# umutdundar99/progressive-stable-diffusion

Measured on AMD Instinct MI355X. Metric: images/sec at 512x512, 50 DDIM steps, bs/GPU=4, higher is better.
Workload: dtype f16; 1 GPU; 512x512, 50 DDIM steps, bs=4/GPU, delta-steer lambda=3.0, routing gates on, conditioning prep + VAE decode included; global_batch=4, parallelism=batch-shard x1 + 1 all-gather of uint8 frames

## Files before the change

progressive-stable-diffusion_amd/csrc/attn2_fused.hip:

```cpp
#include "dadd_common.h"
#include "igemm_args.h"

namespace {

constexpr int BK = 64, NS = 384, BN2 = 160;
constexpr int B1_BYTES = NS * BK * 2;
constexpr int P_STRIDE = 896;
constexpr int B2_BYTES = BN2 * BK * 2;
template <int BM> constexpr int a_bytes() { return BM * BK * 2; }
template <int BM> constexpr int stage1() { return a_bytes<BM>() + B1_BYTES; }
template <int BM> constexpr int p_bytes() { return BM * P_STRIDE; }
template <int BM> constexpr int nst2() { return p_bytes<BM>() + 4 * B2_BYTES <= 160 * 1024 - 1024 ? 4 : 2; }
template <int BM> constexpr int smem_bytes() {
  return (p_bytes<BM>() + nst2<BM>() * B2_BYTES) > 2 * stage1<BM>() ? (p_bytes<BM>() + nst2<BM>() * B2_BYTES) : 2 * stage1<BM>();
}

typedef __attribute__((address_space(3))) void* lptr_t;
constexpr unsigned OOB = 0x80000000u;

struct Attn2Args {
  const half_t* x;
  const half_t* mcat;
  const half_t* vw;
  const float* bias;
  const half_t* residual;
  half_t* out;
  float* ln_stats;
  const float* ln_in;
  const float* ln_c1;
  const float* ln_d;
  float ln_eps;
  int ln_parts;
  int B, HW, C;
};

__device__ __forceinline__ int lds_off(int row, int chunk) {
  return (row * 8 + (chunk ^ ((row >> 1) & 7))) * 8;
}

template <int BM>
__global__ __launch_bounds__(256, 1) void attn2_fused_kernel(const Attn2Args p) {
#if defined(__HIP_DEVICE_COMPILE__)
  constexpr int MI = BM / 32;
  constexpr int WMR = BM / 2;
  constexpr int NXP = BM / 32;
  constexpr int A_BYTES = a_bytes<BM>(), STAGE1 = stage1<BM>(), P_BYTES = p_bytes<BM>();
  extern __shared__ __attribute__((aligned(1024))) char smem[];
  const int t = threadIdx.x, lane = t & 63;
  const int wave = __builtin_amdgcn_readfirstlane(t >> 6);
  const int wm = wave >> 1, wn = wave & 1;
  const int tile = xcd_remap(blockIdx.x, gridDim.x);
  const int m0 = tile * BM;
  const int b = m0 / p.HW;
  const int C = p.C;
  const int nk1 = C / BK;
  const int lrow = lane >> 3, lch = lane & 7;
  const int fq = lane >> 4, mc = lane & 15, g = fq;

  const __amdgpu_buffer_rsrc_t rsX =
      __builtin_amdgcn_make_buffer_rsrc((void*)p.x, 0, (int)((size_t)p.B * p.HW * C * 2), 0x00020000);
  const __amdgpu_buffer_rsrc_t rsM = __builtin_amdgcn_make_buffer_rsrc(
      (void*)(p.mcat + (size_t)b * NS * C), 0, NS * C * 2, 0x00020000);
  unsigned xv[NXP], mv[12];
#pragma unroll
  for (int i = 0; i < NXP; ++i) {
    const int row = (i * 4 + wave) * 8 + lrow;
    xv[i] = (unsigned)(((size_t)(m0 + row) * C + (lch ^ ((row >> 1) & 7)) * 8) * 2);
  }
#pragma unroll
  for (int j = 0; j < 12; ++j) {
    const int row = (j * 4 + wave) * 8 + lrow;
    mv[j] = (unsigned)(((size_t)row * C + (lch ^ ((row >> 1) & 7)) * 8) * 2);
  }
  auto issue1 = [&](int kt, int stage) {
    char* sa = smem + stage * STAGE1 + wave * 1024;
    const unsigned ko = (unsigned)(kt * BK * 2);
#pragma unroll
    for (int i = 0; i < NXP; ++i)
      __builtin_amdgcn_raw_ptr_buffer_load_lds(rsX, (lptr_t)(sa + i * 4096), 16, xv[i], ko, 0, 0);
#pragma unroll
    for (int j = 0; j < 12; ++j)
      __builtin_amdgcn_raw_ptr_buffer_load_lds(rsM, (lptr_t)(sa + A_BYTES + j * 4096), 16, mv[j], ko, 0, 0);
  };

  f4 acc[12][MI];
#pragma unroll
  for (int j = 0; j < 12; ++j)
#pragma unroll
    for (int i = 0; i < MI; ++i) acc[j][i] = f4{0.f, 0.f, 0.f, 0.f};
  const bool fold = p.ln_in != nullptr;
  float lmu[MI], lrs[MI];
#pragma unroll
  for (int i = 0; i < MI; ++i) lmu[i] = 0.f, lrs[i] = 1.f;
  if (fold) {
    const dadd_f2* st = reinterpret_cast<const dadd_f2*>(p.ln_in);
    const size_t mtot = (size_t)p.B * p.HW;
    float sa[MI], sq[MI];
#pragma unroll
    for (int i = 0; i < MI; ++i) sa[i] = sq[i] = 0.f;
    for (int pp = 0; pp < p.ln_parts; ++pp)
#pragma unroll
      for (int i = 0; i < MI; ++i) {
        const dadd_f2 v = st[(size_t)pp * mtot + m0 + wm * WMR + i * 16 + mc];
        sa[i] += v[0];
        sq[i] += v[1];
      }
    const float inv = __builtin_amdgcn_rcpf((float)C);
#pragma unroll
    for (int i = 0; i < MI; ++i) {
      const float mu = sa[i] * inv;
      lmu[i] = mu;
      lrs[i] = rsqrtf(fmaxf(sq[i] * inv - mu * mu, 0.f) + p.ln_eps);
    }
  }
  int fa[2], fb[2];
#pragma unroll
  for (int s = 0; s < 2; ++s) {
    fa[s] = lds_off(wm * WMR + mc, s * 4 + fq) * 2;
    fb[s] = A_BYTES + lds_off(wn * 192 + mc, s * 4 + fq) * 2;
  }
  issue1(0, 0);
  for (int kt = 0; kt < nk1; ++kt) {
    asm volatile("s_waitcnt vmcnt(0)" ::: "memory");
    __syncthreads();
    if (kt + 1 < nk1) issue1(kt + 1, (kt + 1) & 1);
    const char* st = smem + (kt & 1) * STAGE1;
#pragma unroll
    for (int s = 0; s < 2; ++s) {
      h8 xa[MI], wb[12];
#pragma unroll
      for (int i = 0; i < MI; ++i) xa[i] = *reinterpret_cast<const h8*>(st + fa[s] + i * 2048);
#pragma unroll
      for (int j = 0; j < 12; ++j) wb[j] = *reinterpret_cast<const h8*>(st + fb[s] + j * 2048);
#pragma unroll
      for (int j = 0; j < 12; ++j)
#pragma unroll
        for (int i = 0; i < MI; ++i)
          acc[j][i] = __builtin_amdgcn_mfma_f32_16x16x32_f16(wb[j], xa[i], acc[j][i], 0, 0, 0);
    }
  }
  f4 fc1[12], fd[12];
  if (fold) {
#pragma unroll
    for (int j = 0; j < 12; ++j) {
      const int k = wn * 192 + j * 16 + g * 4;
      fc1[j] = *reinterpret_cast<const f4*>(p.ln_c1 + (size_t)b * NS + k);
      fd[j] = *reinterpret_cast<const f4*>(p.ln_d + (size_t)b * NS + k);
    }
  }
  __syncthreads();

  const int nt2 = C / BN2;
  const int nk2 = NS / BK;
  const int n_it2 = nt2 * nk2;
  const __amdgpu_buffer_rsrc_t rsV = __builtin_amdgcn_make_buffer_rsrc(
      (void*)(p.vw + (size_t)b * C * NS), 0, C * NS * 2, 0x00020000);
  unsigned vv[5];
#pragma unroll
  for (int j = 0; j < 5; ++j) {
    const int row = (j * 4 + wave) * 8 + lrow;
    vv[j] = (unsigned)(((size_t)row * NS + (lch ^ ((row >> 1) & 7)) * 8) * 2);
  }
  auto issue2 = [&](int it, int stage) {
    const int nt = it / nk2, kt = it - nt * nk2;
    char* sa = smem + P_BYTES + stage * B2_BYTES + wave * 1024;
    const unsigned so = (unsigned)(((size_t)nt * BN2 * NS + kt * BK) * 2);
#pragma unroll
    for (int j = 0; j < 5; ++j)
      __builtin_amdgcn_raw_ptr_buffer_load_lds(rsV, (lptr_t)(sa + j * 4096), 16, vv[j], so, 0, 0);
  };
  constexpr int NST2 = nst2<BM>();
  issue2(0, 0);
  if constexpr (NST2 == 4) {
    if (1 < n_it2) issue2(1, 1);
    if (2 < n_it2) issue2(2, 2);
  }

#pragma unroll
  for (int i = 0; i < MI; ++i) {
    const int row = wm * WMR + i * 16 + mc;
    char* prow = smem + row * P_STRIDE;
    const int swz = (row >> 1) & 7;
#pragma unroll
    for (int j = 0; j < 12; ++j) {
      f4 v = acc[j][i];
      if (fold) v = lrs[i] * (v - lmu[i] * fc1[j]) + fd[j];
      float mx = fmaxf(fmaxf(v[0], v[1]), fmaxf(v[2], v[3]));
      mx = dadd_max_x16x32(mx);
      const float e0 = __builtin_amdgcn_exp2f(v[0] - mx), e1 = __builtin_amdgcn_exp2f(v[1] - mx);
      const float e2 = __builtin_amdgcn_exp2f(v[2] - mx), e3 = __builtin_amdgcn_exp2f(v[3] - mx);
      float sum = (e0 + e1) + (e2 + e3);
      sum = dadd_sum_x16x32(sum);
      const float inv = __builtin_amdgcn_rcpf(sum);
      const h4 o = {(half_t)(e0 * inv), (half_t)(e1 * inv), (half_t)(e2 * inv), (half_t)(e3 * inv)};
      const int k = wn * 192 + j * 16 + g * 4;
      const int seg = k >> 6, ch = (k & 63) >> 3;
      *reinterpret_cast<h4*>(prow + seg * 128 + ((ch ^ swz) << 4) + (k & 7) * 2) = o;
    }
  }

  const int fp0 = (wm * WMR + mc) * P_STRIDE;
  const int pswz = ((wm * WMR + mc) >> 1) & 7;
  const int swb = wn * 80 + mc;
  const int fv0 = (swb * 8 + (fq ^ ((swb >> 1) & 7))) * 16;
  f4 acc2[5][MI];
  for (int it = 0; it < n_it2; ++it) {
    const int nt = it / nk2, kt = it - nt * nk2;
    if (kt == 0) {
#pragma unroll
      for (int j = 0; j < 5; ++j)
#pragma unroll
        for (int i = 0; i < MI; ++i) acc2[j][i] = f4{0.f, 0.f, 0.f, 0.f};
    }
    if constexpr (NST2 == 4) {
      const int younger = min(2, n_it2 - 1 - it);
      if (younger == 2) asm volatile("s_waitcnt vmcnt(10)" ::: "memory");
      else if (younger == 1) asm volatile("s_waitcnt vmcnt(5)" ::: "memory");
      else asm volatile("s_waitcnt vmcnt(0)" ::: "memory");
    } else {
      asm volatile("s_waitcnt vmcnt(0)" ::: "memory");
    }
    __syncthreads();
    if (it + NST2 - 1 < n_it2) issue2(it + NST2 - 1, (it + NST2 - 1) & (NST2 - 1));
    const char* vt = smem + P_BYTES + (it & (NST2 - 1)) * B2_BYTES;
#pragma unroll
    for (int s = 0; s < 2; ++s) {
      h8 pa[MI], wb[5];
#pragma unroll
      for (int i = 0; i < MI; ++i)
        pa[i] = *reinterpret_cast<const h8*>(smem + fp0 + i * 16 * P_STRIDE + kt * 128 + (((s * 4 + fq) ^ pswz) << 4));
#pragma unroll
      for (int j = 0; j < 5; ++j) wb[j] = *reinterpret_cast<const h8*>(vt + (fv0 ^ (s * 64)) + j * 2048);
#pragma unroll
      for (int j = 0; j < 5; ++j)
#pragma unroll
        for (int i = 0; i < MI; ++i)
          acc2[j][i] = __builtin_amdgcn_mfma_f32_16x16x32_f16(wb[j], pa[i], acc2[j][i], 0, 0, 0);
    }
    if (kt == nk2 - 1) {
      f4 bias4[5];
      h4 res4[5][MI];
#pragma unroll
      for (int j = 0; j < 5; ++j) {
        const int n = nt * BN2 + wn * 80 + j * 16 + g * 4;
        bias4[j] = p.bias ? *reinterpret_cast<const f4*>(p.bias + n) : f4{0.f, 0.f, 0.f, 0.f};
#pragma unroll
        for (int i = 0; i < MI; ++i)
          res4[j][i] = *reinterpret_cast<const h4*>(p.residual + ((size_t)m0 + wm * WMR + i * 16 + mc) * C + n);
      }
#pragma unroll
      for (int i = 0; i < MI; ++i) {
        const size_t m = (size_t)m0 + wm * WMR + i * 16 + mc;
        float rs1 = 0.f, rs2 = 0.f;
#pragma unroll
        for (int j = 0; j < 5; ++j) {
          const int n = nt * BN2 + wn * 80 + j * 16 + g * 4;
          const f4 v = acc2[j][i] + bias4[j];
          const h4 rv = res4[j][i];
          const h4 o = {(half_t)(v[0] + (float)rv[0]), (half_t)(v[1] + (float)rv[1]),
                        (half_t)(v[2] + (float)rv[2]), (half_t)(v[3] + (float)rv[3])};
          *reinterpret_cast<h4*>(p.out + m * C + n) = o;
#pragma unroll
          for (int r = 0; r < 4; ++r) {
            const float f = (float)o[r];
            rs1 += f;
            rs2 = fmaf(f, f, rs2);
          }
        }
        if (p.ln_stats) {
          rs1 = dadd_sum_x16x32(rs1);
          rs2 = dadd_sum_x16x32(rs2);
          if (g == 0)
            reinterpret_cast<dadd_f2*>(p.ln_stats)[(size_t)(nt * 2 + wn) * ((size_t)p.B * p.HW) + m] = dadd_f2{rs1, rs2};
        }
      }
    }
  }
#endif
}

}

int g_attn2_cus = 0;

int dadd_init_attn2_fused() {
  DADD_HIP(hipFuncSetAttribute(reinterpret_cast<const void*>(&attn2_fused_kernel<128>),
                               hipFuncAttributeMaxDynamicSharedMemorySize, smem_bytes<128>()));
  DADD_HIP(hipFuncSetAttribute(reinterpret_cast<const void*>(&attn2_fused_kernel<64>),
                               hipFuncAttributeMaxDynamicSharedMemorySize, smem_bytes<64>()));
  int dev = 0;
  DADD_HIP(hipGetDevice(&dev));
  DADD_HIP(hipDeviceGetAttribute(&g_attn2_cus, hipDeviceAttributeMultiprocessorCount, dev));
  return DADD_OK;
}

extern "C" int dadd_attn2_fused_f16(const void* x, const void* mcat, const void* vw, const float* bias,
                                    const void* residual, void* out, float* ln_stats_out, const float* ln_stats_in,
                                    int ln_parts_in, const float* ln_c1, const float* ln_d, float ln_eps, int B, int HW,
                                    int C, void* stream) {
  DADD_REQUIRE(x && mcat && vw && residual && out, "attn2_fused: null pointer");
  DADD_REQUIRE(B > 0 && HW > 0 && HW % 128 == 0, "attn2_fused: H*W=%d must be a multiple of 128", HW);
  DADD_REQUIRE(C > 0 && C % BN2 == 0 && C % BK == 0, "attn2_fused: C=%d must be a multiple of 320", C);
  DADD_REQUIRE((size_t)B * HW * C * 2 < 0x7FF00000ull, "attn2_fused: activation larger than the 2 GiB buffer window");
  DADD_REQUIRE(dadd_aligned16(x) && dadd_aligned16(mcat) && dadd_aligned16(vw) && dadd_aligned16(residual) &&
                   dadd_aligned16(out) && (!bias || dadd_aligned16(bias)),
// ... 29 lines not shown
```

progressive-stable-diffusion_amd/csrc/elementwise.hip:

```cpp
#include "dadd_common.h"

namespace {

#ifndef DADD_BF16
__global__ __launch_bounds__(256) void pack_kernel(const float* __restrict__ x, half_t* __restrict__ out,
                                                   int B, int C, int HW, float scale,
                                                   const float* __restrict__ mat,
                                                   const float* __restrict__ vec) {
  const size_t total = (size_t)B * HW;
  for (size_t i = (size_t)blockIdx.x * 256 + threadIdx.x; i < total; i += (size_t)gridDim.x * 256) {
    const size_t b = i / HW, pix = i - b * HW;
    float v[8], o[8];
#pragma unroll
    for (int c = 0; c < 8; ++c) v[c] = (c < C) ? x[(b * C + c) * HW + pix] * scale : 0.f;
    if (mat) {
#pragma unroll
      for (int c = 0; c < 8; ++c) {
        float a = 0.f;
        if (c < C) {
          a = vec ? vec[c] : 0.f;
          for (int k = 0; k < C; ++k) a += mat[c * C + k] * v[k];
        }
        o[c] = a;
      }
    } else {
#pragma unroll
      for (int c = 0; c < 8; ++c) o[c] = v[c];
    }
    h8 r;
#pragma unroll
    for (int c = 0; c < 8; ++c) r[c] = (half_t)o[c];
    *reinterpret_cast<h8*>(out + i * 8) = r;
  }
}

__global__ __launch_bounds__(256) void conv_cin8_kernel(const half_t* __restrict__ x,
                                                        const half_t* __restrict__ w,
                                                        const float* __restrict__ bias,
                                                        half_t* __restrict__ out, int B, int H, int W,
                                                        int Cout) {
  const int npix = B * H * W;
  const int pix = blockIdx.x * 256 + threadIdx.x;
  const int co0 = blockIdx.y * 8;
  if (pix >= npix) return;
  const int b = pix / (H * W), rem = pix - b * H * W, oy = rem / W, ox = rem - oy * W;
  float acc[8];
#pragma unroll
  for (int o = 0; o < 8; ++o) acc[o] = bias ? bias[co0 + o] : 0.f;
#pragma unroll
  for (int tap = 0; tap < 9; ++tap) {
    const int iy = oy + tap / 3 - 1, ix = ox + tap % 3 - 1;
    if (iy < 0 || iy >= H || ix < 0 || ix >= W) continue;
    const h8 xv = *reinterpret_cast<const h8*>(x + ((size_t)(b * H + iy) * W + ix) * 8);
#pragma unroll
    for (int o = 0; o < 8; ++o) {
      const h8 wv = *reinterpret_cast<const h8*>(w + ((size_t)(co0 + o) * 9 + tap) * 8);
#pragma unroll
      for (int c = 0; c < 8; ++c) acc[o] += (float)xv[c] * (float)wv[c];
    }
  }
  h8 r;
#pragma unroll
  for (int o = 0; o < 8; ++o) r[o] = (half_t)acc[o];
  *reinterpret_cast<h8*>(out + (size_t)pix * Cout + co0) = r;
}

#endif

__global__ __launch_bounds__(256) void conv_in_nchw_kernel(const float* __restrict__ x, const half_t* __restrict__ w,
                                                           const float* __restrict__ bias, half_t* __restrict__ out,
                                                           int B, int C, int H, int W, int Cout) {
  typedef half_t ci_h2 __attribute__((ext_vector_type(2)));
  const int HW = H * W, npix = B * HW;
  const int pix = blockIdx.x * 256 + threadIdx.x;
  const int co0 = blockIdx.y * 8;
  if (pix >= npix) return;
  const int b = pix / HW, rem = pix - b * HW, oy = rem / W, ox = rem - oy * W;
  ci_h2 x01[9], x23[9];
#pragma unroll
  for (int tap = 0; tap < 9; ++tap) {
    const int iy = oy + tap / 3 - 1, ix = ox + tap % 3 - 1;
    const bool ok = iy >= 0 && iy < H && ix >= 0 && ix < W;
    const float* xp = x + (size_t)b * C * HW + (ok ? iy * W + ix : rem);
    float v[4];
#pragma unroll
    for (int c = 0; c < 4; ++c) v[c] = (c < C && ok) ? xp[(size_t)c * HW] : 0.f;
    x01[tap] = ci_h2{(half_t)v[0], (half_t)v[1]};
    x23[tap] = ci_h2{(half_t)v[2], (half_t)v[3]};
  }
  h8 r;
#pragma unroll
  for (int o = 0; o < 8; ++o) {
    float acc = bias ? bias[co0 + o] : 0.f;
#pragma unroll
    for (int tap = 0; tap < 9; ++tap) {
      const h4 wv = *reinterpret_cast<const h4*>(w + ((size_t)(co0 + o) * 9 + tap) * 8);
      acc = dadd_fdot2(x01[tap], ci_h2{wv[0], wv[1]}, acc);
      acc = dadd_fdot2(x23[tap], ci_h2{wv[2], wv[3]}, acc);
    }
    r[o] = (half_t)acc;
  }
  *reinterpret_cast<h8*>(out + (size_t)pix * Cout + co0) = r;
}

template <int CG>
__global__ __launch_bounds__(256) void conv_in_nchw_gn_kernel(const float* __restrict__ x, const half_t* __restrict__ w,
                                                              const float* __restrict__ bias, half_t* __restrict__ out,
                                                              float* __restrict__ gn_ws, int B, int C, int H, int W, int Cout) {
  typedef half_t ci_h2 __attribute__((ext_vector_type(2)));
  static_assert((4 * CG) % 8 == 0, "four groups must be whole 8-channel stores");
  __shared__ float red[4][8];
  const int HW = H * W;
  const int pix = blockIdx.x * 256 + threadIdx.x;
  const int co0 = blockIdx.y * 4 * CG;
  const int b = pix / HW, rem = pix - b * HW, oy = rem / W, ox = rem - oy * W;
  ci_h2 x01[9], x23[9];
#pragma unroll
  for (int tap = 0; tap < 9; ++tap) {
    const int iy = oy + tap / 3 - 1, ix = ox + tap % 3 - 1;
    const bool ok = iy >= 0 && iy < H && ix >= 0 && ix < W;
    const float* xp = x + (size_t)b * C * HW + (ok ? iy * W + ix : rem);
    float v[4];
#pragma unroll
    for (int c = 0; c < 4; ++c) v[c] = (c < C && ok) ? xp[(size_t)c * HW] : 0.f;
    x01[tap] = ci_h2{(half_t)v[0], (half_t)v[1]};
    x23[tap] = ci_h2{(half_t)v[2], (half_t)v[3]};
  }
  float st[8] = {0.f, 0.f, 0.f, 0.f, 0.f, 0.f, 0.f, 0.f};
#pragma unroll
  for (int o8 = 0; o8 < 4 * CG / 8; ++o8) {
    h8 r;
#pragma unroll
    for (int o = 0; o < 8; ++o) {
      const int co = co0 + o8 * 8 + o;
      float acc = bias ? bias[co] : 0.f;
#pragma unroll
      for (int tap = 0; tap < 9; ++tap) {
        const h4 wv = *reinterpret_cast<const h4*>(w + ((size_t)co * 9 + tap) * 8);
        acc = dadd_fdot2(x01[tap], ci_h2{wv[0], wv[1]}, acc);
        acc = dadd_fdot2(x23[tap], ci_h2{wv[2], wv[3]}, acc);
      }
      r[o] = (half_t)acc;
      const float f = (float)r[o];
      const int g = (o8 * 8 + o) / CG;
      st[2 * g] += f;
      st[2 * g + 1] += f * f;
    }
    *reinterpret_cast<h8*>(out + (size_t)pix * Cout + co0 + o8 * 8) = r;
  }
#pragma unroll
  for (int i = 0; i < 8; ++i) st[i] = wave_sum(st[i]);
  const int lane = threadIdx.x & 63, wave = threadIdx.x >> 6;
  if (lane == 0) {
#pragma unroll
    for (int i = 0; i < 8; ++i) red[wave][i] = st[i];
  }
  __syncthreads();
  if (threadIdx.x < 8) {
    const int i = threadIdx.x;
    const float v = (red[0][i] + red[1][i]) + (red[2][i] + red[3][i]);
    const int chunk = (blockIdx.x * 256 - b * HW) >> 8, nchunk = HW >> 8;
    gn_ws[(((size_t)b * nchunk + chunk) * 32 + blockIdx.y * 4 + (i >> 1)) * 2 + (i & 1)] = v;
  }
}

typedef half_t cc_h2 __attribute__((ext_vector_type(2)));
__global__ __launch_bounds__(256) void conv_cout4_kernel(const half_t* __restrict__ x,
                                                         const half_t* __restrict__ w,
                                                         const float* __restrict__ bias,
                                                         float* __restrict__ out, int B, int H, int W,
                                                         int C, int Cout, int mode,
                                                         const float* __restrict__ coef) {
#pragma clang fp contract(off)
  extern __shared__ __attribute__((aligned(16))) char cc_smem[];
  half_t* ws = reinterpret_cast<half_t*>(cc_smem);
  const int wtot = Cout * 9 * C;
  for (int i = threadIdx.x * 8; i < wtot; i += 256 * 8) *reinterpret_cast<h8*>(ws + i) = *reinterpret_cast<const h8*>(w + i);
  __syncthreads();
  const int npix = B * H * W, HW = H * W;
  const int sub = threadIdx.x & 15;
  const int nchunk = C >> 3;
  int pixs[2], bb[2], oy[2], ox[2];
  bool live[2];
#pragma unroll
  for (int q = 0; q < 2; ++q) {
    int pix = blockIdx.x * 32 + q * 16 + (threadIdx.x >> 4);
    live[q] = pix < npix;
    if (!live[q]) pix = npix - 1;
    pixs[q] = pix;
    bb[q] = pix / HW;
    const int rem = pix - bb[q] * HW;
    oy[q] = rem / W;
    ox[q] = rem - oy[q] * W;
  }
  float a0[4] = {0.f, 0.f, 0.f, 0.f}, a1[4] = {0.f, 0.f, 0.f, 0.f};
  const h8 zero8 = {0, 0, 0, 0, 0, 0, 0, 0};
  for (int ch = sub; ch < nchunk; ch += 16) {
    h8 xv[2][9];
#pragma unroll
    for (int q = 0; q < 2; ++q)
#pragma unroll
      for (int tap = 0; tap < 9; ++tap) {
        const int iy = oy[q] + tap / 3 - 1, ix = ox[q] + tap % 3 - 1;
        const bool ok = iy >= 0 && iy < H && ix >= 0 && ix < W;
        const half_t* xp = x + ((size_t)(bb[q] * H + (ok ? iy : oy[q])) * W + (ok ? ix : ox[q])) * C + ch * 8;
        const h8 v = *reinterpret_cast<const h8*>(xp);
        xv[q][tap] = ok ? v : zero8;
      }
#pragma unroll
    for (int tap = 0; tap < 9; ++tap)
#pragma unroll
      for (int o = 0; o < 4; ++o) {
        if (o < Cout) {
          const h8 wv = *reinterpret_cast<const h8*>(ws + (o * 9 + tap) * C + ch * 8);
#pragma unroll
          for (int c = 0; c < 4; ++c) {
            const cc_h2 wp = {wv[2 * c], wv[2 * c + 1]};
            a0[o] = dadd_fdot2(cc_h2{xv[0][tap][2 * c], xv[0][tap][2 * c + 1]}, wp, a0[o]);
            a1[o] = dadd_fdot2(cc_h2{xv[1][tap][2 * c], xv[1][tap][2 * c + 1]}, wp, a1[o]);
          }
        }
      }
  }
#pragma unroll
  for (int o = 0; o < 4; ++o) {
#pragma unroll
    for (int s = 8; s > 0; s >>= 1) {
      a0[o] += __shfl_xor(a0[o], s, 64);
      a1[o] += __shfl_xor(a1[o], s, 64);
    }
  }
#pragma unroll
  for (int q = 0; q < 2; ++q) {
    if (live[q] && sub < Cout) {
      float v = q ? a1[0] : a0[0];
      if (sub == 1) v = q ? a1[1] : a0[1];
      if (sub == 2) v = q ? a1[2] : a0[2];
      if (sub == 3) v = q ? a1[3] : a0[3];
      v += bias ? bias[sub] : 0.f;
      if (mode == 1) {
        v = fminf(fmaxf(v, -1.f), 1.f);
        v = (v + 1.f) / 2.f;
        v = fminf(fmaxf(v, 0.f), 1.f);
      } else if (mode == 2) {
        v = fminf(fmaxf(v, -30.f), 20.f);
      }
      float* dst = out + ((size_t)bb[q] * Cout + sub) * HW + (pixs[q] - bb[q] * HW);
      if (mode == 3) {
        const float c0 = coef[0], c1 = coef[1], c2 = coef[2], c3 = coef[3];
        const float sx = c1 * v;
        const float num = *dst - sx;
        float x0 = num / c0;
        x0 = fminf(fmaxf(x0, -4.0f), 4.0f);
        const float ta = c2 * x0;
        const float tb = c3 * v;
        v = (c2 < 0.f) ? x0 : ta + tb;
      }
      *dst = v;
    }
  }
}

#ifndef DADD_BF16
__global__ void timestep_features_kernel(const int64_t* __restrict__ t, float* __restrict__ out, int M,
                                         int dim) {
  const int half = dim / 2;
  const int i = blockIdx.x * blockDim.x + threadIdx.x;
  if (i >= M * half) return;
  const int m = i / half, j = i - m * half;
  const float freq = expf(-9.210340371976184f * (float)j / (float)half);
  const float ang = (float)t[m] * freq;
  out[(size_t)m * dim + j] = cosf(ang);
  out[(size_t)m * dim + half + j] = sinf(ang);
}

__device__ __forceinline__ float rows_act(float v, int act) {
  return act == 1 ? dadd_silu(v) : (act == 2 ? 0.5f * v * (1.0f + erff(v * 0.70710678118654752440f)) : v);
}
__device__ __forceinline__ void rows_load8(const half_t* p, float (&o)[8]) {
  const h8 v = *reinterpret_cast<const h8*>(p);
#pragma unroll
  for (int c = 0; c < 8; ++c) o[c] = (float)v[c];
}
__device__ __forceinline__ void rows_load8(const float* p, float (&o)[8]) {
  const f4 a = *reinterpret_cast<const f4*>(p), b = *reinterpret_cast<const f4*>(p + 4);
#pragma unroll
  for (int c = 0; c < 4; ++c) { o[c] = a[c]; o[c + 4] = b[c]; }
}

template <typename WT>
__global__ __launch_bounds__(256) void linear_rows_kernel(const float* __restrict__ x,
                                                          const WT* __restrict__ w,
                                                          const float* __restrict__ bias,
                                                          float* __restrict__ out, int M, int K, int N,
                                                          int act_in, int act_out) {
  extern __shared__ float xs[];
  const int lane = threadIdx.x & 63;
  const int n = blockIdx.x * 4 + (threadIdx.x >> 6);
  const int nchunk = K >> 3;
  for (int m0 = 0; m0 < M; m0 += 8) {
    const int mr = min(8, M - m0);
    __syncthreads();
    for (int i = threadIdx.x; i < mr * K; i += 256) {
      xs[i] = rows_act(x[(size_t)m0 * K + i], act_in);
    }
// ... 326 lines not shown
```

progressive-stable-diffusion_amd/csrc/norm.hip:

```cpp
#include "dadd_common.h"

namespace {

constexpr int GN_MAXV = 2;
constexpr float GN_FAR = 256.f;

struct GnArgs {
  const half_t* x1;
  const half_t* x2;
  const float* gamma;
  const float* beta;
  half_t* out;
  float* ws;
  float* stats;
  int C1, C2, C, HW, groups, cg, nchunk, rows_per_chunk, rows_per_block, TV, RP, silu;
  float eps;
};

__device__ __forceinline__ h8 gn_load(const GnArgs& p, size_t pix, int c) {
  return (c < p.C1) ? *reinterpret_cast<const h8*>(p.x1 + pix * p.C1 + c)
                    : *reinterpret_cast<const h8*>(p.x2 + pix * p.C2 + (c - p.C1));
}

__global__ __launch_bounds__(256) void gn_stats_kernel(const GnArgs p) {
  extern __shared__ float sm[];
  const int t = threadIdx.x, tv = t % p.TV, tr = t / p.TV;
  const int b = blockIdx.y, chunk = blockIdx.x;
  const int row0 = chunk * p.rows_per_chunk;
  const int row1 = min(p.HW, row0 + p.rows_per_chunk);
  float s[GN_MAXV][8], ss[GN_MAXV][8];
#pragma unroll
  for (int u = 0; u < GN_MAXV; ++u)
#pragma unroll
    for (int e = 0; e < 8; ++e) s[u][e] = ss[u][e] = 0.f;
  const int nvec = p.C >> 3;
  if (tr < p.RP) {
    for (int row = row0 + tr; row < row1; row += 4 * p.RP) {
      h8 xv[4][GN_MAXV];
#pragma unroll
      for (int q = 0; q < 4; ++q) {
        const int rr = row + q * p.RP;
        const size_t pix = (size_t)b * p.HW + (rr < row1 ? rr : row);
#pragma unroll
        for (int u = 0; u < GN_MAXV; ++u) {
          const int v = tv + u * p.TV;
          if (v < nvec) xv[q][u] = gn_load(p, pix, v * 8);
        }
      }
#pragma unroll
      for (int q = 0; q < 4; ++q) {
        if (row + q * p.RP >= row1) continue;
#pragma unroll
        for (int u = 0; u < GN_MAXV; ++u) {
          if (tv + u * p.TV < nvec) {
#pragma unroll
            for (int e = 0; e < 8; ++e) {
              const float f = (float)xv[q][u][e];
              s[u][e] += f;
              ss[u][e] += f * f;
            }
          }
        }
      }
    }
#pragma unroll
    for (int u = 0; u < GN_MAXV; ++u) {
      const int v = tv + u * p.TV;
      if (v < nvec) {
#pragma unroll
        for (int e = 0; e < 8; ++e) {
          sm[tr * p.C + v * 8 + e] = s[u][e];
          sm[(p.RP + tr) * p.C + v * 8 + e] = ss[u][e];
        }
      }
    }
  }
  __syncthreads();
  {
    const int g = t >> 3, sub = t & 7;
    float a = 0.f, q = 0.f;
    if (g < p.groups) {
      const int n = p.RP * p.cg;
      for (int idx = sub; idx < n; idx += 8) {
        const int r = idx / p.cg, c = g * p.cg + (idx - r * p.cg);
        a += sm[r * p.C + c];
        q += sm[(p.RP + r) * p.C + c];
      }
    }
#pragma unroll
    for (int o = 4; o > 0; o >>= 1) {
      a += __shfl_xor(a, o, 64);
      q += __shfl_xor(q, o, 64);
    }
    if (g < p.groups && sub == 0) {
      float* w = p.ws + (((size_t)b * p.nchunk + chunk) * p.groups + g) * 2;
      w[0] = a;
      w[1] = q;
    }
  }
}

template <bool FIN>
__global__ __launch_bounds__(256) void gn_apply_kernel(const GnArgs p) {
  extern __shared__ float sm[];
  float* scale = sm;
  float* shift = sm + p.C;
  const int t = threadIdx.x, tv = t % p.TV, tr = t / p.TV;
  const int b = blockIdx.y;
  const float* st = p.stats + (size_t)b * p.groups * 2;
  if (FIN) {
    float* lst = sm + 2 * p.C;
    const int g = t >> 3, sub = t & 7;
    double a = 0.0, q = 0.0;
    if (g < p.groups) {
      for (int k = sub; k < p.nchunk; k += 32) {
        float2 v[4];
#pragma unroll
        for (int u = 0; u < 4; ++u) {
          const int kk = k + 8 * u;
          v[u] = kk < p.nchunk ? *reinterpret_cast<const float2*>(p.ws + (((size_t)b * p.nchunk + kk) * p.groups + g) * 2)
                               : float2{0.f, 0.f};
        }
#pragma unroll
        for (int u = 0; u < 4; ++u) {
          a += (double)v[u].x;
          q += (double)v[u].y;
        }
      }
    }
#pragma unroll
    for (int o = 4; o > 0; o >>= 1) {
      a += __shfl_xor(a, o, 64);
      q += __shfl_xor(q, o, 64);
    }
    if (g < p.groups && sub == 0) {
      const double n = (double)p.HW * (double)p.cg;
      const double mu = a / n;
      double var = q / n - mu * mu;
      if (var < 0.0) var = 0.0;
      lst[2 * g] = (float)mu;
      lst[2 * g + 1] = (float)(1.0 / sqrt(var + (double)p.eps));
    }
    __syncthreads();
    st = lst;
  }
  for (int c = t; c < p.C; c += 256) {
    const int g = c / p.cg;
    const float sc = st[2 * g + 1] * p.gamma[c];
    scale[c] = sc;
    shift[c] = p.beta[c] - st[2 * g] * sc;
  }
  __syncthreads();
  if (tr >= p.RP) return;
  const int nvec = p.C >> 3;
  const int row0 = blockIdx.x * p.rows_per_block;
  const int row1 = min(p.HW, row0 + p.rows_per_block);
  float sc[GN_MAXV][8], sh[GN_MAXV][8];
  bool far = false;
#pragma unroll
  for (int u = 0; u < GN_MAXV; ++u) {
    const int v = tv + u * p.TV;
#pragma unroll
    for (int e = 0; e < 8; ++e) {
      sc[u][e] = v < nvec ? scale[v * 8 + e] : 0.f;
      sh[u][e] = v < nvec ? shift[v * 8 + e] : 0.f;
      far |= fabsf(sh[u][e]) > GN_FAR;
    }
  }
  if (far) {
    for (int row = row0 + tr; row < row1; row += p.RP) {
      const size_t pix = (size_t)b * p.HW + row;
#pragma unroll 1
      for (int u = 0; u < GN_MAXV; ++u) {
        const int v = tv + u * p.TV;
        if (v >= nvec) continue;
        const h8 xv = gn_load(p, pix, v * 8);
        h8 o;
#pragma unroll
        for (int e = 0; e < 8; ++e) {
          const int c = v * 8 + e;
          float f = ((float)xv[e] - st[2 * (c / p.cg)]) * scale[c] + p.beta[c];
          if (p.silu) f = dadd_silu(f);
          o[e] = (half_t)f;
        }
        *reinterpret_cast<h8*>(p.out + pix * p.C + v * 8) = o;
      }
    }
    return;
  }
  for (int row = row0 + tr; row < row1; row += 4 * p.RP) {
    h8 xv[4][GN_MAXV];
#pragma unroll
    for (int q = 0; q < 4; ++q) {
      const int rr = row + q * p.RP;
      const size_t pix = (size_t)b * p.HW + (rr < row1 ? rr : row);
#pragma unroll
      for (int u = 0; u < GN_MAXV; ++u)
        if (tv + u * p.TV < nvec) xv[q][u] = gn_load(p, pix, (tv + u * p.TV) * 8);
    }
#pragma unroll
    for (int q = 0; q < 4; ++q) {
      const int rr = row + q * p.RP;
      if (rr >= row1) continue;
      const size_t pix = (size_t)b * p.HW + rr;
#pragma unroll
      for (int u = 0; u < GN_MAXV; ++u) {
        const int v = tv + u * p.TV;
        if (v < nvec) {
          h8 o;
#pragma unroll
          for (int e = 0; e < 8; ++e) {
            float f = (float)xv[q][u][e] * sc[u][e] + sh[u][e];
            if (p.silu) f = dadd_silu(f);
            o[e] = (half_t)f;
          }
          *reinterpret_cast<h8*>(p.out + pix * p.C + v * 8) = o;
        }
      }
    }
  }
}

__global__ __launch_bounds__(256) void gn_fused_kernel(const GnArgs p) {
  extern __shared__ __attribute__((aligned(16))) char smraw[];
  h2* slab = reinterpret_cast<h2*>(smraw);
  __shared__ float red[2][4];
  const int t = threadIdx.x, lane = t & 63, wave = t >> 6;
  const int g = blockIdx.x, b = blockIdx.y;
  const int hp = p.cg >> 1;
  const int c0 = g * p.cg;
  const int npair = p.HW * hp;
  float s = 0.f, ss = 0.f;
  for (int idx = t; idx < npair; idx += 256) {
    const int row = idx / hp, cp = idx - row * hp;
    const int c = c0 + 2 * cp;
    const size_t pix = (size_t)b * p.HW + row;
    const h2 v = (c < p.C1) ? *reinterpret_cast<const h2*>(p.x1 + pix * p.C1 + c)
                            : *reinterpret_cast<const h2*>(p.x2 + pix * p.C2 + (c - p.C1));
    slab[idx] = v;
    const float a = (float)v[0], d = (float)v[1];
    s += a + d;
    ss += a * a + d * d;
  }
  s = wave_sum(s);
  ss = wave_sum(ss);
  if (lane == 0) { red[0][wave] = s; red[1][wave] = ss; }
  __syncthreads();
  const double n = (double)p.HW * (double)p.cg;
  const double sum = (double)red[0][0] + (double)red[0][1] + (double)red[0][2] + (double)red[0][3];
  const double sq = (double)red[1][0] + (double)red[1][1] + (double)red[1][2] + (double)red[1][3];
  const double mu = sum / n;
  double var = sq / n - mu * mu;
  if (var < 0.0) var = 0.0;
  const float mean = (float)mu, rstd = (float)(1.0 / sqrt(var + (double)p.eps));
  for (int idx = t; idx < npair; idx += 256) {
    const int row = idx / hp, cp = idx - row * hp;
    const int c = c0 + 2 * cp;
    const h2 v = slab[idx];
    h2 o;
#pragma unroll
    for (int e = 0; e < 2; ++e) {
      const float sc = rstd * p.gamma[c + e];
      float f = ((float)v[e] - mean) * sc + p.beta[c + e];
      if (p.silu) f = dadd_silu(f);
      o[e] = (half_t)f;
    }
    *reinterpret_cast<h2*>(p.out + ((size_t)b * p.HW + row) * p.C + c) = o;
  }
}

constexpr int GN_CHUNK_MAX = 64;
constexpr int GN_FUSED_MAX_BYTES = 16 * 1024;

constexpr int LN_MAXV = 4;
__global__ __launch_bounds__(256) void layernorm_kernel(const half_t* __restrict__ x,
                                                        const float* __restrict__ gamma,
                                                        const float* __restrict__ beta,
                                                        half_t* __restrict__ out, int M, int C,
                                                        float eps) {
  const int lane = threadIdx.x & 63;
  const int row = blockIdx.x * 4 + (threadIdx.x >> 6);
  if (row >= M) return;
  const int nvec = C >> 3;
  const half_t* xr = x + (size_t)row * C;
  h8 v[LN_MAXV];
  float sum = 0.f;
#pragma unroll
  for (int u = 0; u < LN_MAXV; ++u) {
    const int i = lane + 64 * u;
    if (i < nvec) {
      v[u] = *reinterpret_cast<const h8*>(xr + i * 8);
#pragma unroll
      for (int e = 0; e < 8; ++e) sum += (float)v[u][e];
    }
  }
  const float mean = wave_sum(sum) / (float)C;
  float sq = 0.f;
#pragma unroll
  for (int u = 0; u < LN_MAXV; ++u) {
    const int i = lane + 64 * u;
    if (i < nvec) {
#pragma unroll
// ... 129 lines not shown
```

Before: 11.32 images/sec.

## Deepen attn2 phase-1 ring and prefetch loads ahead of barriers in conv/GN kernels

The attn2 fused kernel's first GEMM phase moves from a 2-stage BK=64 double buffer to a 4-stage BK=32 ring with partial vmcnt waits and a new swizzle, reusing the phase-2 LDS allocation. Several elementwise kernels (conv_in, conv_out, GN apply) now issue their global input loads, weight loads and gamma/beta/stats prefetches before shared-memory setup and barriers, so load latency overlaps the setup. conv_in also stages its weights and bias in LDS instead of reading them per output. These changes target latency stalls on memory, at the cost of more registers held live and more intricate synchronisation.

```diff
diff --git a/progressive-stable-diffusion_amd/csrc/attn2_fused.hip b/progressive-stable-diffusion_amd/csrc/attn2_fused.hip
--- a/progressive-stable-diffusion_amd/csrc/attn2_fused.hip
+++ b/progressive-stable-diffusion_amd/csrc/attn2_fused.hip
@@ -4,16 +4,16 @@
 namespace {
 
 constexpr int BK = 64, NS = 384, BN2 = 160;
-constexpr int B1_BYTES = NS * BK * 2;
+constexpr int BK1 = 32, NST1 = 4;
+constexpr int B1_BYTES = NS * BK1 * 2;
 constexpr int P_STRIDE = 896;
 constexpr int B2_BYTES = BN2 * BK * 2;
-template <int BM> constexpr int a_bytes() { return BM * BK * 2; }
+template <int BM> constexpr int a_bytes() { return BM * BK1 * 2; }
 template <int BM> constexpr int stage1() { return a_bytes<BM>() + B1_BYTES; }
 template <int BM> constexpr int p_bytes() { return BM * P_STRIDE; }
 template <int BM> constexpr int nst2() { return p_bytes<BM>() + 4 * B2_BYTES <= 160 * 1024 - 1024 ? 4 : 2; }
-template <int BM> constexpr int smem_bytes() {
-  return (p_bytes<BM>() + nst2<BM>() * B2_BYTES) > 2 * stage1<BM>() ? (p_bytes<BM>() + nst2<BM>() * B2_BYTES) : 2 * stage1<BM>();
-}
+template <int BM> constexpr int smem_bytes() { return p_bytes<BM>() + nst2<BM>() * B2_BYTES; }
+static_assert(NST1 * stage1<64>() <= smem_bytes<64>() && NST1 * stage1<128>() <= smem_bytes<128>(), "phase-1 ring exceeds the LDS allocation");
 
 typedef __attribute__((address_space(3))) void* lptr_t;
 constexpr unsigned OOB = 0x80000000u;
@@ -34,8 +34,20 @@
   int B, HW, C;
 };
 
-__device__ __forceinline__ int lds_off(int row, int chunk) {
-  return (row * 8 + (chunk ^ ((row >> 1) & 7))) * 8;
+__device__ __forceinline__ int swz1(int row) { return (0 - (row >> 2)) & 3; }
+__device__ __forceinline__ int lds_off1(int row, int chunk) {
+  return row * 64 + ((chunk ^ swz1(row)) << 4);
+}
+
+template <int D>
+__device__ __forceinline__ void ring_sync(int younger) {
+  static_assert(2 * D <= 63, "vmcnt is a 6-bit counter");
+  if (younger >= 2) asm volatile("s_waitcnt vmcnt(%0) lgkmcnt(0)" ::"n"(2 * D) : "memory");
+  else if (younger == 1) asm volatile("s_waitcnt vmcnt(%0) lgkmcnt(0)" ::"n"(D) : "memory");
+  else asm volatile("s_waitcnt vmcnt(0) lgkmcnt(0)" ::: "memory");
+  __builtin_amdgcn_s_barrier();
+  asm volatile("" ::: "memory");
+  __builtin_amdgcn_sched_barrier(0);
 }
 
 template <int BM>
@@ -43,7 +55,10 @@
 #if defined(__HIP_DEVICE_COMPILE__)
   constexpr int MI = BM / 32;
   constexpr int WMR = BM / 2;
-  constexpr int NXP = BM / 32;
+  constexpr int NXP = BM / 64;
+  constexpr int NMP = NS / 64;
+  constexpr int D1 = NXP + NMP, D2 = 5;
+  static_assert(2 * D1 <= 63 && 2 * D2 <= 63, "vmcnt is a 6-bit counter");
   constexpr int A_BYTES = a_bytes<BM>(), STAGE1 = stage1<BM>(), P_BYTES = p_bytes<BM>();
   extern __shared__ __attribute__((aligned(1024))) char smem[];
   const int t = threadIdx.x, lane = t & 63;
@@ -53,33 +68,34 @@
   const int m0 = tile * BM;
   const int b = m0 / p.HW;
   const int C = p.C;
-  const int nk1 = C / BK;
+  const int nk1 = C / BK1;
   const int lrow = lane >> 3, lch = lane & 7;
+  const int lrow1 = lane >> 2, lch1 = lane & 3;
   const int fq = lane >> 4, mc = lane & 15, g = fq;
 
   const __amdgpu_buffer_rsrc_t rsX =
       __builtin_amdgcn_make_buffer_rsrc((void*)p.x, 0, (int)((size_t)p.B * p.HW * C * 2), 0x00020000);
   const __amdgpu_buffer_rsrc_t rsM = __builtin_amdgcn_make_buffer_rsrc(
       (void*)(p.mcat + (size_t)b * NS * C), 0, NS * C * 2, 0x00020000);
-  unsigned xv[NXP], mv[12];
+  unsigned xv[NXP], mv[NMP];
 #pragma unroll
   for (int i = 0; i < NXP; ++i) {
-    const int row = (i * 4 + wave) * 8 + lrow;
-    xv[i] = (unsigned)(((size_t)(m0 + row) * C + (lch ^ ((row >> 1) & 7)) * 8) * 2);
-  }
-#pragma unroll
-  for (int j = 0; j < 12; ++j) {
-    const int row = (j * 4 + wave) * 8 + lrow;
-    mv[j] = (unsigned)(((size_t)row * C + (lch ^ ((row >> 1) & 7)) * 8) * 2);
+    const int row = (i * 4 + wave) * 16 + lrow1;
+    xv[i] = (unsigned)(((size_t)(m0 + row) * C + (lch1 ^ swz1(row)) * 8) * 2);
+  }
+#pragma unroll
+  for (int j = 0; j < NMP; ++j) {
+    const int row = (j * 4 + wave) * 16 + lrow1;
+    mv[j] = (unsigned)(((size_t)row * C + (lch1 ^ swz1(row)) * 8) * 2);
   }
   auto issue1 = [&](int kt, int stage) {
     char* sa = smem + stage * STAGE1 + wave * 1024;
-    const unsigned ko = (unsigned)(kt * BK * 2);
+    const unsigned ko = (unsigned)(kt * BK1 * 2);
 #pragma unroll
     for (int i = 0; i < NXP; ++i)
       __builtin_amdgcn_raw_ptr_buffer_load_lds(rsX, (lptr_t)(sa + i * 4096), 16, xv[i], ko, 0, 0);
 #pragma unroll
-    for (int j = 0; j < 12; ++j)
+    for (int j = 0; j < NMP; ++j)
       __builtin_amdgcn_raw_ptr_buffer_load_lds(rsM, (lptr_t)(sa + A_BYTES + j * 4096), 16, mv[j], ko, 0, 0);
   };
 
@@ -113,31 +129,25 @@
       lrs[i] = rsqrtf(fmaxf(sq[i] * inv - mu * mu, 0.f) + p.ln_eps);
     }
   }
-  int fa[2], fb[2];
-#pragma unroll
-  for (int s = 0; s < 2; ++s) {
-    fa[s] = lds_off(wm * WMR + mc, s * 4 + fq) * 2;
-    fb[s] = A_BYTES + lds_off(wn * 192 + mc, s * 4 + fq) * 2;
-  }
+  const int fa = lds_off1(wm * WMR + mc, fq);
+  const int fb = A_BYTES + lds_off1(wn * 192 + mc, fq);
   issue1(0, 0);
+  if (1 < nk1) issue1(1, 1);
+  if (2 < nk1) issue1(2, 2);
   for (int kt = 0; kt < nk1; ++kt) {
-    asm volatile("s_waitcnt vmcnt(0)" ::: "memory");
-    __syncthreads();
-    if (kt + 1 < nk1) issue1(kt + 1, (kt + 1) & 1);
-    const char* st = smem + (kt & 1) * STAGE1;
-#pragma unroll
-    for (int s = 0; s < 2; ++s) {
-      h8 xa[MI], wb[12];
-#pragma unroll
-      for (int i = 0; i < MI; ++i) xa[i] = *reinterpret_cast<const h8*>(st + fa[s] + i * 2048);
-#pragma unroll
-      for (int j = 0; j < 12; ++j) wb[j] = *reinterpret_cast<const h8*>(st + fb[s] + j * 2048);
-#pragma unroll
-      for (int j = 0; j < 12; ++j)
-#pragma unroll
-        for (int i = 0; i < MI; ++i)
-          acc[j][i] = __builtin_amdgcn_mfma_f32_16x16x32_f16(wb[j], xa[i], acc[j][i], 0, 0, 0);
-    }
+    ring_sync<D1>(min(2, nk1 - 1 - kt));
+    if (kt + NST1 - 1 < nk1) issue1(kt + NST1 - 1, (kt + NST1 - 1) & (NST1 - 1));
+    const char* st = smem + (kt & (NST1 - 1)) * STAGE1;
+    h8 xa[MI], wb[12];
+#pragma unroll
+    for (int i = 0; i < MI; ++i) xa[i] = *reinterpret_cast<const h8*>(st + fa + i * 1024);
+#pragma unroll
+    for (int j = 0; j < 12; ++j) wb[j] = *reinterpret_cast<const h8*>(st + fb + j * 1024);
+#pragma unroll
+    for (int j = 0; j < 12; ++j)
+#pragma unroll
+      for (int i = 0; i < MI; ++i)
+        acc[j][i] = __builtin_amdgcn_mfma_f32_16x16x32_f16(wb[j], xa[i], acc[j][i], 0, 0, 0);
   }
   f4 fc1[12], fd[12];
   if (fold) {
@@ -148,7 +158,10 @@
       fd[j] = *reinterpret_cast<const f4*>(p.ln_d + (size_t)b * NS + k);
     }
   }
-  __syncthreads();
+  asm volatile("s_waitcnt lgkmcnt(0)" ::: "memory");
+  __builtin_amdgcn_s_barrier();
+  asm volatile("" ::: "memory");
+  __builtin_amdgcn_sched_barrier(0);
 
   const int nt2 = C / BN2;
   const int nk2 = NS / BK;
@@ -212,15 +225,7 @@
 #pragma unroll
         for (int i = 0; i < MI; ++i) acc2[j][i] = f4{0.f, 0.f, 0.f, 0.f};
     }
-    if constexpr (NST2 == 4) {
-      const int younger = min(2, n_it2 - 1 - it);
-      if (younger == 2) asm volatile("s_waitcnt vmcnt(10)" ::: "memory");
-      else if (younger == 1) asm volatile("s_waitcnt vmcnt(5)" ::: "memory");
-      else asm volatile("s_waitcnt vmcnt(0)" ::: "memory");
-    } else {
-      asm volatile("s_waitcnt vmcnt(0)" ::: "memory");
-    }
-    __syncthreads();
+    ring_sync<D2>(NST2 == 4 ? min(2, n_it2 - 1 - it) : 0);
     if (it + NST2 - 1 < n_it2) issue2(it + NST2 - 1, (it + NST2 - 1) & (NST2 - 1));
     const char* vt = smem + P_BYTES + (it & (NST2 - 1)) * B2_BYTES;
 #pragma unroll
diff --git a/progressive-stable-diffusion_amd/csrc/elementwise.hip b/progressive-stable-diffusion_amd/csrc/elementwise.hip
--- a/progressive-stable-diffusion_amd/csrc/elementwise.hip
+++ b/progressive-stable-diffusion_amd/csrc/elementwise.hip
@@ -67,6 +67,29 @@
 
 #endif
 
+template <typename H2>
+__device__ __forceinline__ void conv_in_load_taps(const float* __restrict__ xb, int C, int H, int W, int oy, int ox,
+                                                  H2 (&x01)[9], H2 (&x23)[9]) {
+  const size_t HW = (size_t)H * W;
+  float v[9][4];
+#pragma unroll
+  for (int tap = 0; tap < 9; ++tap) {
+    const int iy = min(max(oy + tap / 3 - 1, 0), H - 1), ix = min(max(ox + tap % 3 - 1, 0), W - 1);
+    const float* xp = xb + iy * W + ix;
+#pragma unroll
+    for (int c = 0; c < 4; ++c) v[tap][c] = xp[(c < C ? c : 0) * HW];
+  }
+#pragma unroll
+  for (int tap = 0; tap < 9; ++tap) {
+    const int iy = oy + tap / 3 - 1, ix = ox + tap % 3 - 1;
+    const bool ok = iy >= 0 && iy < H && ix >= 0 && ix < W;
+#pragma unroll
+    for (int c = 0; c < 4; ++c) v[tap][c] = (c < C && ok) ? v[tap][c] : 0.f;
+    x01[tap] = H2{(half_t)v[tap][0], (half_t)v[tap][1]};
+    x23[tap] = H2{(half_t)v[tap][2], (half_t)v[tap][3]};
+  }
+}
+
 __global__ __launch_bounds__(256) void conv_in_nchw_kernel(const float* __restrict__ x, const half_t* __restrict__ w,
                                                            const float* __restrict__ bias, half_t* __restrict__ out,
                                                            int B, int C, int H, int W, int Cout) {
@@ -77,17 +100,7 @@
   if (pix >= npix) return;
   const int b = pix / HW, rem = pix - b * HW, oy = rem / W, ox = rem - oy * W;
   ci_h2 x01[9], x23[9];
-#pragma unroll
-  for (int tap = 0; tap < 9; ++tap) {
-    const int iy = oy + tap / 3 - 1, ix = ox + tap % 3 - 1;
-    const bool ok = iy >= 0 && iy < H && ix >= 0 && ix < W;
-    const float* xp = x + (size_t)b * C * HW + (ok ? iy * W + ix : rem);
-    float v[4];
-#pragma unroll
-    for (int c = 0; c < 4; ++c) v[c] = (c < C && ok) ? xp[(size_t)c * HW] : 0.f;
-    x01[tap] = ci_h2{(half_t)v[0], (half_t)v[1]};
-    x23[tap] = ci_h2{(half_t)v[2], (half_t)v[3]};
-  }
+  conv_in_load_taps(x + (size_t)b * C * HW, C, H, W, oy, ox, x01, x23);
   h8 r;
 #pragma unroll
   for (int o = 0; o < 8; ++o) {
@@ -109,36 +122,41 @@
                                                               float* __restrict__ gn_ws, int B, int C, int H, int W, int Cout) {
   typedef half_t ci_h2 __attribute__((ext_vector_type(2)));
   static_assert((4 * CG) % 8 == 0, "four groups must be whole 8-channel stores");
+  ci_h2 x01[9], x23[9];
   __shared__ float red[4][8];
+  __shared__ uint4 wl[4 * CG][5];
+  __shared__ float bl[4 * CG];
   const int HW = H * W;
   const int pix = blockIdx.x * 256 + threadIdx.x;
   const int co0 = blockIdx.y * 4 * CG;
-  const int b = pix / HW, rem = pix - b * HW, oy = rem / W, ox = rem - oy * W;
-  ci_h2 x01[9], x23[9];
-#pragma unroll
-  for (int tap = 0; tap < 9; ++tap) {
-    const int iy = oy + tap / 3 - 1, ix = ox + tap % 3 - 1;
-    const bool ok = iy >= 0 && iy < H && ix >= 0 && ix < W;
-    const float* xp = x + (size_t)b * C * HW + (ok ? iy * W + ix : rem);
-    float v[4];
-#pragma unroll
-    for (int c = 0; c < 4; ++c) v[c] = (c < C && ok) ? xp[(size_t)c * HW] : 0.f;
-    x01[tap] = ci_h2{(half_t)v[0], (half_t)v[1]};
-    x23[tap] = ci_h2{(half_t)v[2], (half_t)v[3]};
-  }
+  {
+    const int e = threadIdx.x < 4 * CG * 5 ? threadIdx.x : 0, o = e / 5, k = e - o * 5;
+    const uint2* wp = reinterpret_cast<const uint2*>(w + ((size_t)(co0 + o) * 9 + 2 * k) * 8);
+    const uint2 lo = wp[0], hi = wp[k < 4 ? 2 : 0];
+    const float bv = bias ? bias[co0 + (threadIdx.x < 4 * CG ? threadIdx.x : 0)] : 0.f;
+    const int b = pix / HW, rem = pix - b * HW, oy = rem / W, ox = rem - oy * W;
+    conv_in_load_taps(x + (size_t)b * C * HW, C, H, W, oy, ox, x01, x23);
+    if (threadIdx.x < 4 * CG * 5) wl[o][k] = uint4{lo.x, lo.y, k < 4 ? hi.x : 0u, k < 4 ? hi.y : 0u};
+    if (threadIdx.x < 4 * CG) bl[threadIdx.x] = bv;
+  }
+  __syncthreads();
+  const int b = pix / HW;
   float st[8] = {0.f, 0.f, 0.f, 0.f, 0.f, 0.f, 0.f, 0.f};
 #pragma unroll
   for (int o8 = 0; o8 < 4 * CG / 8; ++o8) {
     h8 r;
 #pragma unroll
     for (int o = 0; o < 8; ++o) {
-      const int co = co0 + o8 * 8 + o;
-      float acc = bias ? bias[co] : 0.f;
-#pragma unroll
-      for (int tap = 0; tap < 9; ++tap) {
-        const h4 wv = *reinterpret_cast<const h4*>(w + ((size_t)co * 9 + tap) * 8);
-        acc = dadd_fdot2(x01[tap], ci_h2{wv[0], wv[1]}, acc);
-        acc = dadd_fdot2(x23[tap], ci_h2{wv[2], wv[3]}, acc);
+      float acc = bl[o8 * 8 + o];
+#pragma unroll
+      for (int k = 0; k < 5; ++k) {
+        const uint4 q = wl[o8 * 8 + o][k];
+        acc = dadd_fdot2(x01[2 * k], __builtin_bit_cast(ci_h2, q.x), acc);
+        acc = dadd_fdot2(x23[2 * k], __builtin_bit_cast(ci_h2, q.y), acc);
+        if (k < 4) {
+          acc = dadd_fdot2(x01[2 * k + 1], __builtin_bit_cast(ci_h2, q.z), acc);
+          acc = dadd_fdot2(x23[2 * k + 1], __builtin_bit_cast(ci_h2, q.w), acc);
+        }
       }
       r[o] = (half_t)acc;
       const float f = (float)r[o];
@@ -175,8 +193,6 @@
   extern __shared__ __attribute__((aligned(16))) char cc_smem[];
   half_t* ws = reinterpret_cast<half_t*>(cc_smem);
   const int wtot = Cout * 9 * C;
-  for (int i = threadIdx.x * 8; i < wtot; i += 256 * 8) *reinterpret_cast<h8*>(ws + i) = *reinterpret_cast<const h8*>(w + i);
-  __syncthreads();
   const int npix = B * H * W, HW = H * W;
   const int sub = threadIdx.x & 15;
   const int nchunk = C >> 3;
@@ -195,20 +211,46 @@
   }
   float a0[4] = {0.f, 0.f, 0.f, 0.f}, a1[4] = {0.f, 0.f, 0.f, 0.f};
   const h8 zero8 = {0, 0, 0, 0, 0, 0, 0, 0};
+  h8 xv[2][9];
+  auto tap_ok = [&](int q, int tap) {
+    const int iy = oy[q] + tap / 3 - 1, ix = ox[q] + tap % 3 - 1;
+    return iy >= 0 && iy < H && ix >= 0 && ix < W;
+  };
+  auto load_tap = [&](int q, int tap, int ch) {
+    const int iy = oy[q] + tap / 3 - 1, ix = ox[q] + tap % 3 - 1;
+    const bool ok = tap_ok(q, tap);
+    const half_t* xp = x + ((size_t)(bb[q] * H + (ok ? iy : oy[q])) * W + (ok ? ix : ox[q])) * C + ch * 8;
+    xv[q][tap] = *reinterpret_cast<const h8*>(xp);
+  };
+  constexpr int WB = 6;
+  h8 wr[WB];
+#pragma unroll
+  for (int u = 0; u < WB; ++u) {
+    const int i = (threadIdx.x + u * 256) * 8;
+    wr[u] = *reinterpret_cast<const h8*>(w + (i < wtot ? i : 0));
+  }
+  {
+    const int ch0 = sub < nchunk ? sub : 0;
+#pragma unroll
+    for (int tap = 0; tap < 9; ++tap) {
+      load_tap(0, tap, ch0);
+      load_tap(1, tap, ch0);
+    }
+  }
+#pragma unroll
+  for (int u = 0; u < WB; ++u) {
+    const int i = (threadIdx.x + u * 256) * 8;
+    if (i < wtot) *reinterpret_cast<h8*>(ws + i) = wr[u];
+  }
+  for (int i = (threadIdx.x + WB * 256) * 8; i < wtot; i += 256 * 8) *reinterpret_cast<h8*>(ws + i) = *reinterpret_cast<const h8*>(w + i);
+  __syncthreads();
   for (int ch = sub; ch < nchunk; ch += 16) {
-    h8 xv[2][9];
-#pragma unroll
-    for (int q = 0; q < 2; ++q)
-#pragma unroll
-      for (int tap = 0; tap < 9; ++tap) {
-        const int iy = oy[q] + tap / 3 - 1, ix = ox[q] + tap % 3 - 1;
-        const bool ok = iy >= 0 && iy < H && ix >= 0 && ix < W;
-        const half_t* xp = x + ((size_t)(bb[q] * H + (ok ? iy : oy[q])) * W + (ok ? ix : ox[q])) * C + ch * 8;
-        const h8 v = *reinterpret_cast<const h8*>(xp);
-        xv[q][tap] = ok ? v : zero8;
-      }
-#pragma unroll
-    for (int tap = 0; tap < 9; ++tap)
+    const int chn = ch + 16 < nchunk ? ch + 16 : ch;
+#pragma unroll
+    for (int tap = 0; tap < 9; ++tap) {
+      const h8 x0 = tap_ok(0, tap) ? xv[0][tap] : zero8, x1 = tap_ok(1, tap) ? xv[1][tap] : zero8;
+      load_tap(0, tap, chn);
+      load_tap(1, tap, chn);
 #pragma unroll
       for (int o = 0; o < 4; ++o) {
         if (o < Cout) {
@@ -216,11 +258,12 @@
 #pragma unroll
           for (int c = 0; c < 4; ++c) {
             const cc_h2 wp = {wv[2 * c], wv[2 * c + 1]};
-            a0[o] = dadd_fdot2(cc_h2{xv[0][tap][2 * c], xv[0][tap][2 * c + 1]}, wp, a0[o]);
-            a1[o] = dadd_fdot2(cc_h2{xv[1][tap][2 * c], xv[1][tap][2 * c + 1]}, wp, a1[o]);
+            a0[o] = dadd_fdot2(cc_h2{x0[2 * c], x0[2 * c + 1]}, wp, a0[o]);
+            a1[o] = dadd_fdot2(cc_h2{x1[2 * c], x1[2 * c + 1]}, wp, a1[o]);
           }
         }
       }
+    }
   }
 #pragma unroll
   for (int o = 0; o < 4; ++o) {
diff --git a/progressive-stable-diffusion_amd/csrc/norm.hip b/progressive-stable-diffusion_amd/csrc/norm.hip
--- a/progressive-stable-diffusion_amd/csrc/norm.hip
+++ b/progressive-stable-diffusion_amd/csrc/norm.hip
@@ -22,6 +22,17 @@
                     : *reinterpret_cast<const h8*>(p.x2 + pix * p.C2 + (c - p.C1));
 }
 
+__device__ __forceinline__ void gn_load_rows(const GnArgs& p, int b, int row, int row1, int tv, int nvec, h8 (&xv)[4][GN_MAXV]) {
+#pragma unroll
+  for (int q = 0; q < 4; ++q) {
+    const int rr = row + q * p.RP;
+    const size_t pix = (size_t)b * p.HW + (rr < row1 ? rr : row);
+#pragma unroll
+    for (int u = 0; u < GN_MAXV; ++u)
+      if (tv + u * p.TV < nvec) xv[q][u] = gn_load(p, pix, (tv + u * p.TV) * 8);
+  }
+}
+
 __global__ __launch_bounds__(256) void gn_stats_kernel(const GnArgs p) {
   extern __shared__ float sm[];
   const int t = threadIdx.x, tv = t % p.TV, tr = t / p.TV;
@@ -108,9 +119,36 @@
   const int t = threadIdx.x, tv = t % p.TV, tr = t / p.TV;
   const int b = blockIdx.y;
   const float* st = p.stats + (size_t)b * p.groups * 2;
+  const int nvec = p.C >> 3;
+  const int row0 = blockIdx.x * p.rows_per_block;
+  const int row1 = min(p.HW, row0 + p.rows_per_block);
+  constexpr int GN_PRE = 4;
+  const int g0 = t >> 3, sub = t & 7;
+  float2 vf[4];
+  if (FIN) {
+    const int gc = g0 < p.groups ? g0 : 0;
+#pragma unroll
+    for (int u = 0; u < 4; ++u) {
+      const int kk = sub + 8 * u;
+      vf[u] = *reinterpret_cast<const float2*>(p.ws + (((size_t)b * p.nchunk + (kk < p.nchunk ? kk : 0)) * p.groups + gc) * 2);
+    }
+  }
+  float gpre[GN_PRE], bpre[GN_PRE];
+#pragma unroll
+  for (int u = 0; u < GN_PRE; ++u) {
+    const int c = t + 256 * u;
+    gpre[u] = p.gamma[c < p.C ? c : 0];
+    bpre[u] = p.beta[c < p.C ? c : 0];
+  }
+  const int rowf = row0 + tr;
+  h8 xf[4][GN_MAXV];
+  {
+    const bool mine = tr < p.RP && rowf < row1;
+    gn_load_rows(p, b, mine ? rowf : row0, mine ? row1 : row0 + 1, mine ? tv : 0, nvec, xf);
+  }
   if (FIN) {
     float* lst = sm + 2 * p.C;
-    const int g = t >> 3, sub = t & 7;
+    const int g = g0;
     double a = 0.0, q = 0.0;
     if (g < p.groups) {
       for (int k = sub; k < p.nchunk; k += 32) {
@@ -118,8 +156,11 @@
 #pragma unroll
         for (int u = 0; u < 4; ++u) {
           const int kk = k + 8 * u;
-          v[u] = kk < p.nchunk ? *reinterpret_cast<const float2*>(p.ws + (((size_t)b * p.nchunk + kk) * p.groups + g) * 2)
-                               : float2{0.f, 0.f};
+          if (k == sub)
+            v[u] = kk < p.nchunk ? vf[u] : float2{0.f, 0.f};
+          else
+            v[u] = kk < p.nchunk ? *reinterpret_cast<const float2*>(p.ws + (((size_t)b * p.nchunk + kk) * p.groups + g) * 2)
+                                 : float2{0.f, 0.f};
         }
 #pragma unroll
         for (int u = 0; u < 4; ++u) {
@@ -144,7 +185,17 @@
     __syncthreads();
     st = lst;
   }
-  for (int c = t; c < p.C; c += 256) {
+#pragma unroll
+  for (int u = 0; u < GN_PRE; ++u) {
+    const int c = t + 256 * u;
+    if (c < p.C) {
+      const int g = c / p.cg;
+      const float sc = st[2 * g + 1] * gpre[u];
+      scale[c] = sc;
+      shift[c] = bpre[u] - st[2 * g] * sc;
+    }
+  }
+  for (int c = t + 256 * GN_PRE; c < p.C; c += 256) {
     const int g = c / p.cg;
     const float sc = st[2 * g + 1] * p.gamma[c];
     scale[c] = sc;
@@ -152,23 +203,15 @@
   }
   __syncthreads();
   if (tr >= p.RP) return;
-  const int nvec = p.C >> 3;
-  const int row0 = blockIdx.x * p.rows_per_block;
-  const int row1 = min(p.HW, row0 + p.rows_per_block);
-  float sc[GN_MAXV][8], sh[GN_MAXV][8];
   bool far = false;
 #pragma unroll
   for (int u = 0; u < GN_MAXV; ++u) {
     const int v = tv + u * p.TV;
 #pragma unroll
-    for (int e = 0; e < 8; ++e) {
-      sc[u][e] = v < nvec ? scale[v * 8 + e] : 0.f;
-      sh[u][e] = v < nvec ? shift[v * 8 + e] : 0.f;
-      far |= fabsf(sh[u][e]) > GN_FAR;
-    }
+    for (int e = 0; e < 8; ++e) far |= fabsf(v < nvec ? shift[v * 8 + e] : 0.f) > GN_FAR;
   }
   if (far) {
-    for (int row = row0 + tr; row < row1; row += p.RP) {
+    for (int row = rowf; row < row1; row += p.RP) {
       const size_t pix = (size_t)b * p.HW + row;
 #pragma unroll 1
       for (int u = 0; u < GN_MAXV; ++u) {
@@ -188,36 +231,39 @@
     }
     return;
   }
-  for (int row = row0 + tr; row < row1; row += 4 * p.RP) {
+  auto apply_rows = [&](int row, const h8 (&xv)[4][GN_MAXV]) {
+#pragma unroll
+    for (int u = 0; u < GN_MAXV; ++u) {
+      const int v = tv + u * p.TV;
+      if (v >= nvec) continue;
+      float sc[8], sh[8];
+#pragma unroll
+      for (int e = 0; e < 8; ++e) {
+        sc[e] = scale[v * 8 + e];
+        sh[e] = shift[v * 8 + e];
+      }
+#pragma unroll
+      for (int q = 0; q < 4; ++q) {
+        const int rr = row + q * p.RP;
+        if (rr >= row1) continue;
+        const size_t pix = (size_t)b * p.HW + rr;
+        h8 o;
+#pragma unroll
+        for (int e = 0; e < 8; ++e) {
+          float f = (float)xv[q][u][e] * sc[e] + sh[e];
+          if (p.silu) f = dadd_silu(f);
+          o[e] = (half_t)f;
+        }
+        *reinterpret_cast<h8*>(p.out + pix * p.C + v * 8) = o;
+      }
+    }
+  };
+  if (rowf >= row1) return;
+  apply_rows(rowf, xf);
+  for (int row = rowf + 4 * p.RP; row < row1; row += 4 * p.RP) {
     h8 xv[4][GN_MAXV];
-#pragma unroll
-    for (int q = 0; q < 4; ++q) {
-      const int rr = row + q * p.RP;
-      const size_t pix = (size_t)b * p.HW + (rr < row1 ? rr : row);
-#pragma unroll
-      for (int u = 0; u < GN_MAXV; ++u)
-        if (tv + u * p.TV < nvec) xv[q][u] = gn_load(p, pix, (tv + u * p.TV) * 8);
-    }
-#pragma unroll
-    for (int q = 0; q < 4; ++q) {
-      const int rr = row + q * p.RP;
-      if (rr >= row1) continue;
-      const size_t pix = (size_t)b * p.HW + rr;
-#pragma unroll
-      for (int u = 0; u < GN_MAXV; ++u) {
-        const int v = tv + u * p.TV;
-        if (v < nvec) {
-          h8 o;
-#pragma unroll
-          for (int e = 0; e < 8; ++e) {
-            float f = (float)xv[q][u][e] * sc[u][e] + sh[u][e];
-            if (p.silu) f = dadd_silu(f);
-            o[e] = (half_t)f;
-          }
-          *reinterpret_cast<h8*>(p.out + pix * p.C + v * 8) = o;
-        }
-      }
-    }
+    gn_load_rows(p, b, row, row1, tv, nvec, xv);
+    apply_rows(row, xv);
   }
 }
 
```

After: 11.40 images/sec, median of 6. Within noise of the previous version (+0.7%).
